# facebookresearch/sam-audio

Measured on AMD Instinct MI355X. Metric: seconds-of-audio separated/sec/node, higher is better.
Workload: dtype fp16x3 (fp32 storage as the reference; every big contraction on IEEE-half hi + lo split operands: 3 MFMA products per multiply, fp32 accumulation - fp32-grade results on the 16-bit matrix cores)

## Files before the change

### sam_audio_amd/csrc/common.h

```cpp
#pragma once
#include <hip/hip_runtime.h>
#include <stdint.h>

namespace sa {

struct bf16_t {
  unsigned short v;
};

#ifdef SA_OPERAND_FP16
__device__ __forceinline__ float bf2f(unsigned short h) { return (float)__builtin_bit_cast(_Float16, h); }
__device__ __forceinline__ unsigned short f2bf(float f) {
  return __builtin_bit_cast(unsigned short, (_Float16)f);
}
__device__ __forceinline__ float h16_lo(unsigned w) { return bf2f((unsigned short)(w & 0xffffu)); }
__device__ __forceinline__ float h16_hi(unsigned w) { return bf2f((unsigned short)(w >> 16)); }
typedef __attribute__((ext_vector_type(8))) _Float16 h16x8_t;
#define SA_MFMA_16x16x32(a, b, c) __builtin_amdgcn_mfma_f32_16x16x32_f16(a, b, c, 0, 0, 0)
#define SA_MFMA_32x32x16(a, b, c) __builtin_amdgcn_mfma_f32_32x32x16_f16(a, b, c, 0, 0, 0)
#else
__device__ __forceinline__ float bf2f(unsigned short h) { return __uint_as_float(((unsigned)h) << 16); }
#ifdef SA_BF16_HW_ROUND
__device__ __forceinline__ unsigned short f2bf(float f) { return __builtin_bit_cast(unsigned short, (__bf16)f); }
#else
__device__ __forceinline__ unsigned short f2bf(float f) {
  unsigned u = __float_as_uint(f);
  u += 0x7fffu + ((u >> 16) & 1u);
  return (unsigned short)(u >> 16);
}
#endif
__device__ __forceinline__ float h16_lo(unsigned w) { return __uint_as_float(w << 16); }
__device__ __forceinline__ float h16_hi(unsigned w) { return __uint_as_float(w & 0xffff0000u); }
typedef __attribute__((ext_vector_type(8))) __bf16 h16x8_t;
#define SA_MFMA_16x16x32(a, b, c) __builtin_amdgcn_mfma_f32_16x16x32_bf16(a, b, c, 0, 0, 0)
#define SA_MFMA_32x32x16(a, b, c) __builtin_amdgcn_mfma_f32_32x32x16_bf16(a, b, c, 0, 0, 0)
#endif

typedef __attribute__((ext_vector_type(2))) float f32x2_t;
#ifdef SA_OPERAND_FP16
typedef __attribute__((ext_vector_type(2))) _Float16 h16x2_t;
#else
typedef __attribute__((ext_vector_type(2))) __bf16 h16x2_t;
#endif
__device__ __forceinline__ unsigned pack_h16x2(float a, float b) {
  const f32x2_t v = {a, b};
  return __builtin_bit_cast(unsigned, __builtin_convertvector(v, h16x2_t));
}

#ifdef SA_OPERAND_FP16
constexpr float kH16Max = 65504.f;
#else
constexpr float kH16Max = 3.3895313892515355e38f;
#endif

__device__ __forceinline__ float clamp_h16(float x) { return fminf(fmaxf(x, -kH16Max), kH16Max); }
struct H16Split { unsigned hi, lo; };
__device__ __forceinline__ H16Split split_h16x2(float v0, float v1) {
#pragma clang fp contract(off)
  const unsigned hi = pack_h16x2(clamp_h16(v0), clamp_h16(v1));
  return H16Split{hi, pack_h16x2(v0 - h16_lo(hi), v1 - h16_hi(hi))};
}

struct alt16_t {
  unsigned short v;
};
typedef __attribute__((ext_vector_type(2))) __bf16 alt16x2_t;
typedef __attribute__((ext_vector_type(8))) __bf16 alt16x8_t;
__device__ __forceinline__ unsigned pack_alt16x2(float a, float b) {
  const f32x2_t v = {a, b};
  return __builtin_bit_cast(unsigned, __builtin_convertvector(v, alt16x2_t));
}
__device__ __forceinline__ unsigned short f2alt(float f) { return (unsigned short)(pack_alt16x2(f, 0.f) & 0xffffu); }
#define SA_MFMA_16x16x32_ALT(a, b, c) \
  __builtin_amdgcn_mfma_f32_16x16x32_bf16(__builtin_bit_cast(alt16x8_t, a), __builtin_bit_cast(alt16x8_t, b), c, 0, 0, 0)

template <typename T> struct Elem;
template <> struct Elem<float> {
  static __device__ __forceinline__ float load(const float* p) { return *p; }
  static __device__ __forceinline__ void store(float* p, float v) { *p = v; }
};
template <> struct Elem<bf16_t> {
  static __device__ __forceinline__ float load(const bf16_t* p) { return bf2f(p->v); }
  static __device__ __forceinline__ void store(bf16_t* p, float v) { p->v = f2bf(v); }
};

template <typename T> __device__ __forceinline__ void store4(T* p, float a, float b, float c, float d);
template <> __device__ __forceinline__ void store4<float>(float* p, float a, float b, float c, float d) {
  *(float4*)p = make_float4(a, b, c, d);
}
template <> __device__ __forceinline__ void store4<bf16_t>(bf16_t* p, float a, float b, float c, float d) {
  ushort4 v;
  v.x = f2bf(a); v.y = f2bf(b); v.z = f2bf(c); v.w = f2bf(d);
  *(ushort4*)p = v;
}
template <> __device__ __forceinline__ void store4<alt16_t>(alt16_t* p, float a, float b, float c, float d) {
  *(uint2*)p = make_uint2(pack_alt16x2(a, b), pack_alt16x2(c, d));
}
template <typename T> __device__ __forceinline__ void load2(const T* p, float& a, float& b);
template <> __device__ __forceinline__ void load2<float>(const float* p, float& a, float& b) {
  float2 v = *(const float2*)p; a = v.x; b = v.y;
}
template <> __device__ __forceinline__ void load2<bf16_t>(const bf16_t* p, float& a, float& b) {
  ushort2 v = *(const ushort2*)p; a = bf2f(v.x); b = bf2f(v.y);
}
template <typename T> __device__ __forceinline__ void store2(T* p, float a, float b);
template <> __device__ __forceinline__ void store2<float>(float* p, float a, float b) { *(float2*)p = make_float2(a, b); }
template <> __device__ __forceinline__ void store2<bf16_t>(bf16_t* p, float a, float b) { *(unsigned*)p = pack_h16x2(a, b); }

__device__ __forceinline__ float silu_f(float x) { return x / (1.0f + __expf(-x)); }
__device__ __forceinline__ float gelu_f(float x) { return 0.5f * x * (1.0f + erff(x * 0.7071067811865476f)); }
__device__ __forceinline__ float quick_gelu_f(float x) { return x / (1.0f + __expf(-1.702f * x)); }
__device__ __forceinline__ float relu_f(float x) { return fmaxf(x, 0.f); }
__device__ __forceinline__ float gelu_tanh_f(float x) {
  return 0.5f * x * (1.0f + tanhf(0.7978845608028654f * (x + 0.044715f * x * x * x)));
}
__device__ __forceinline__ float snake_f(float x, float a) {
  float s = sinf(a * x);
  return x + s * s / (a + 1e-9f);
}
__device__ __forceinline__ float snake16_f(float x, float a) {
  const float s = __sinf(a * x);
  return x + s * s * __builtin_amdgcn_rcpf(a + 1e-9f);
}

template <int CTRL> __device__ __forceinline__ float dpp_mov(float v) {
  return __int_as_float(__builtin_amdgcn_update_dpp(0, __float_as_int(v), CTRL, 0xf, 0xf, false));
}
__device__ __forceinline__ float row16_max(float v) {
  v = fmaxf(v, dpp_mov<0x128>(v));
  v = fmaxf(v, dpp_mov<0x124>(v));
  v = fmaxf(v, dpp_mov<0x122>(v));
  v = fmaxf(v, dpp_mov<0x121>(v));
  return v;
}
__device__ __forceinline__ float row16_sum(float v) {
  v += dpp_mov<0x128>(v);
  v += dpp_mov<0x124>(v);
  v += dpp_mov<0x122>(v);
  v += dpp_mov<0x121>(v);
  return v;
}

__device__ __forceinline__ float wave_sum(float v) {
// ... 64 lines not shown
```

### sam_audio_amd/csrc/gemm.hip

```cpp
#include "common.h"
#include "kernels.h"

#include <type_traits>

namespace sa {

typedef h16x8_t bf16x8_t;
typedef __attribute__((ext_vector_type(4))) float f32x4_t;

template <typename T> struct Mma;
template <> struct Mma<bf16_t> {
  typedef bf16x8_t frag_t;
  static __device__ __forceinline__ f32x4_t run(const frag_t& a, const frag_t& b, f32x4_t c) {
    return SA_MFMA_16x16x32(a, b, c);
  }
};
template <> struct Mma<float> {
  typedef f32x4_t frag_t;
  static __device__ __forceinline__ f32x4_t run(const frag_t& a, const frag_t& b, f32x4_t c) {
    c = __builtin_amdgcn_mfma_f32_16x16x4f32(a[0], b[0], c, 0, 0, 0);
    c = __builtin_amdgcn_mfma_f32_16x16x4f32(a[1], b[1], c, 0, 0, 0);
    c = __builtin_amdgcn_mfma_f32_16x16x4f32(a[2], b[2], c, 0, 0, 0);
    c = __builtin_amdgcn_mfma_f32_16x16x4f32(a[3], b[3], c, 0, 0, 0);
    return c;
// ... 17 lines not shown
  __builtin_amdgcn_global_load_lds((const __attribute__((address_space(1))) void*)gsrc,
                                   (__attribute__((address_space(3))) void*)lds_wave_base, 16, 0, 0);
}

template <typename T, int BM, int BN, int WM_, int WN_, bool FLY = false>
__global__ __launch_bounds__(256, (FLY ? 2 : 1)) void gemm_kernel(const GemmParams p) {
  constexpr int NW = WM_ * WN_;
  static_assert(NW == 4, "4 waves per workgroup");
  constexpr int CH = 16 / (int)sizeof(T);
  constexpr int BK = 128 / (int)sizeof(T);
  constexpr int WTM = BM / WM_, WTN = BN / WN_;
  constexpr int FM = WTM / 16, FN = WTN / 16;
  constexpr int AI = BM / 32, BI = BN / 32;
  static_assert(BM % 32 == 0 && BN % 32 == 0 && WTM % 16 == 0 && WTN % 16 == 0, "tile shape");
  constexpr int TILE_A = BM * 128, TILE_B = BN * 128, STAGE = TILE_A + TILE_B;
  constexpr int NS = 2;
  __shared__ __attribute__((aligned(16))) char smem[NS * STAGE];

  const int tid = threadIdx.x;
  const int lane = tid & 63;
  const int wave = __builtin_amdgcn_readfirstlane(tid >> 6);
  const int wm = wave / WN_, wn = wave % WN_;

  const int tiles_n = (p.N + BN - 1) / BN;
  const int tiles_m = (p.M + BM - 1) / BM;
  int id = blockIdx.x;
  const int tn = id % tiles_n;
  id /= tiles_n;
  const int tm = id % tiles_m;
  const int b = id / tiles_m;
  const int m0 = tm * BM, n0 = tn * BN;

  const int r8 = lane >> 3;
  const int chunk = (lane & 7) ^ ((4 * (wave & 1) + (r8 >> 1)) & 7);
  const T* a_rows[AI];
  const T* w_rows[BI];
  {
    const T* A = (const T*)p.A + p.a_off + (long)b * p.a_bstride;
#pragma unroll
    for (int i = 0; i < AI; ++i) {
      int m = m0 + (wave + 4 * i) * 8 + r8;
      m = m < p.M ? m : p.M - 1;
      a_rows[i] = A + (long)m * p.lda;
    }
    const T* W = (const T*)p.W + (long)b * p.w_bstride;
#pragma unroll
    for (int i = 0; i < BI; ++i) {
      int n = n0 + (wave + 4 * i) * 8 + r8;
      n = n < p.N ? n : p.N - 1;
      w_rows[i] = W + (long)n * p.K + chunk * CH;
    }
  }
  int a_in = chunk * CH;
  long a_tap = 0;
  while (a_in >= p.kc) { a_in -= p.kc; a_tap += p.tap_stride; }

  auto issue = [&](int stage) {
    char* sA = smem + stage * STAGE;
    char* sB = sA + TILE_A;
#pragma unroll
    for (int i = 0; i < AI; ++i) dma16(a_rows[i] + a_tap + a_in, sA + (wave + 4 * i) * 1024);
#pragma unroll
    for (int i = 0; i < BI; ++i) dma16(w_rows[i], sB + (wave + 4 * i) * 1024);
    a_in += BK;
    while (a_in >= p.kc) { a_in -= p.kc; a_tap += p.tap_stride; }
#pragma unroll
    for (int i = 0; i < BI; ++i) w_rows[i] += BK;
  };

  f32x4_t acc[FM][FN];
#pragma unroll
  for (int i = 0; i < FM; ++i)
#pragma unroll
    for (int j = 0; j < FN; ++j) acc[i][j] = f32x4_t{0.f, 0.f, 0.f, 0.f};

  const int nslab = p.K / BK;
  const int lr = lane & 15, lg = lane >> 4;
  const int qa = gemm_quant_a(p.flags), qw = gemm_quant_w(p.flags);
  const bool x3fly = FLY || (sizeof(T) == 4 && (p.flags & GEMM_FLAG_X3_FLY) != 0);
  const bool wfly = FLY || (p.flags & GEMM_FLAG_W_FLY16) != 0;
  auto fly_slab = [&](const char* sA, const char* sB) {
#pragma clang fp contract(off)
        bf16x8_t ah[FM], al[FM], bh[FN], bl[FN];
        auto cl = [](float x) { return __builtin_amdgcn_fmed3f(x, -kH16Max, kH16Max); };
        auto split = [&](const char* base, int row, bf16x8_t& hi, bf16x8_t& lo) {
          const int sw = (row >> 1) & 7;
          const f32x4_t v0 = *(const f32x4_t*)(base + row * 128 + ((lg ^ sw) << 4));
          const f32x4_t v1 = *(const f32x4_t*)(base + row * 128 + (((4 + lg) ^ sw) << 4));
          unsigned h[4], l[4];
          h[0] = pack_h16x2(cl(v0[0]), cl(v0[1]));
          h[1] = pack_h16x2(cl(v0[2]), cl(v0[3]));
          h[2] = pack_h16x2(cl(v1[0]), cl(v1[1]));
          h[3] = pack_h16x2(cl(v1[2]), cl(v1[3]));
          l[0] = pack_h16x2(v0[0] - h16_lo(h[0]), v0[1] - h16_hi(h[0]));
          l[1] = pack_h16x2(v0[2] - h16_lo(h[1]), v0[3] - h16_hi(h[1]));
          l[2] = pack_h16x2(v1[0] - h16_lo(h[2]), v1[1] - h16_hi(h[2]));
          l[3] = pack_h16x2(v1[2] - h16_lo(h[3]), v1[3] - h16_hi(h[3]));
          typedef __attribute__((ext_vector_type(4))) unsigned u32x4_t;
          hi = __builtin_bit_cast(bf16x8_t, (u32x4_t){h[0], h[1], h[2], h[3]});
          lo = __builtin_bit_cast(bf16x8_t, (u32x4_t){l[0], l[1], l[2], l[3]});
        };
        if (wfly) {
#pragma unroll
          for (int j = 0; j < FN; ++j) {
            const int row = wn * WTN + j * 16 + lr, sw = (row >> 1) & 7;
            bh[j] = *(const bf16x8_t*)(sB + row * 128 + ((lg ^ sw) << 4));
            bl[j] = *(const bf16x8_t*)(sB + row * 128 + (((4 + lg) ^ sw) << 4));
          }
        } else {
#pragma unroll
          for (int j = 0; j < FN; ++j) split(sB, wn * WTN + j * 16 + lr, bh[j], bl[j]);
        }
#pragma unroll
        for (int i = 0; i < FM; ++i) split(sA, wm * WTM + i * 16 + lr, ah[i], al[i]);
#pragma unroll
        for (int i = 0; i < FM; ++i)
#pragma unroll
          for (int j = 0; j < FN; ++j) acc[i][j] = SA_MFMA_16x16x32(bh[j], al[i], acc[i][j]);
#pragma unroll
        for (int i = 0; i < FM; ++i)
#pragma unroll
          for (int j = 0; j < FN; ++j) acc[i][j] = SA_MFMA_16x16x32(bl[j], ah[i], acc[i][j]);
#pragma unroll
        for (int i = 0; i < FM; ++i)
#pragma unroll
          for (int j = 0; j < FN; ++j) acc[i][j] = SA_MFMA_16x16x32(bh[j], ah[i], acc[i][j]);
  };
  issue(0);
  for (int s = 0; s < nslab; ++s) {
    asm volatile("s_waitcnt vmcnt(0)" ::: "memory");
    __syncthreads();
    if (s + 1 < nslab) issue((s + 1) & 1);
    const char* sA = smem + (s & 1) * STAGE;
    const char* sB = sA + TILE_A;
    if constexpr (sizeof(T) == 4) {
      if (x3fly) {
        fly_slab(sA, sB);
        continue;
      }
    }
    if constexpr (!FLY) {
#pragma unroll
    for (int ks = 0; ks < 2; ++ks) {
      typename Mma<T>::frag_t af[FM], bfr[FN];
      const int c = ks * 4 + lg;
#pragma unroll
      for (int i = 0; i < FM; ++i) {
        const int row = wm * WTM + i * 16 + lr;
        af[i] = *(const typename Mma<T>::frag_t*)(sA + row * 128 + ((c ^ ((row >> 1) & 7)) << 4));
      }
#pragma unroll
      for (int j = 0; j < FN; ++j) {
        const int row = wn * WTN + j * 16 + lr;
        bfr[j] = *(const typename Mma<T>::frag_t*)(sB + row * 128 + ((c ^ ((row >> 1) & 7)) << 4));
      }
      if constexpr (sizeof(T) == 4) {
        if (qa) {
#pragma unroll
          for (int i = 0; i < FM; ++i) af[i] = quant16x4(af[i], qa);
        }
        if (qw) {
#pragma unroll
          for (int j = 0; j < FN; ++j) bfr[j] = quant16x4(bfr[j], qw);
        }
      }
#pragma unroll
      for (int i = 0; i < FM; ++i)
#pragma unroll
        for (int j = 0; j < FN; ++j) acc[i][j] = Mma<T>::run(bfr[j], af[i], acc[i][j]);
    }
    }
  }

  const long bM = (long)b * p.M;
  const int n_out = p.swiglu ? p.N >> 1 : p.N;
  auto finish = [&](float v, const float bias, const float gate, const float res, const float sa, float& a) -> float {
    v += bias;
    if (p.gate) v *= gate;
    v *= p.alpha;
    v += res;
    a = v;
    if (p.act == ACT_SNAKE) a = snake_f(v, sa);
    else if (p.act == ACT_TANH) a = tanhf(v);
// ... 130 lines not shown
static hipError_t launch_cfg(const GemmParams& p, hipStream_t st) {
  const long tiles = (long)((p.M + BM - 1) / BM) * ((p.N + BN - 1) / BN) * p.nbatch;
  hipLaunchKernelGGL((gemm_kernel<T, BM, BN, WM_, WN_>), dim3((unsigned)tiles), dim3(256), 0, st, p);
  return hipGetLastError();
}

static int g_force = -1;
void gemm_force_variant(int v) { g_force = v; }

const char* gemm_variant_name(int v, bool is_bf16) {
  const GemmVariantRow* r = gemm_variant_row(v);
  return !r ? "" : is_bf16 ? r->name16 : r->name32;
}

static GemmVariant gemm1_variant(const GemmParams& p) {
  const int N = p.N;
  if (p.swiglu) return GV_GEMM_128x128;
  if (N <= 32 || N == 96) return GV_GEMM_128x32;
  if (N <= 64 || (N % 128 != 0 && N % 64 == 0 && N <= 448)) return GV_GEMM_128x64;
  const long t128 = (long)((p.M + 127) / 128) * ((N + 127) / 128) * p.nbatch;
  if (t128 < 192) return 2 * t128 < 192 ? GV_GEMM_128x32 : GV_GEMM_128x64;
  return GV_GEMM_128x128;
}
static GemmVariant fly_variant(const GemmParams& p) {
  if (p.N <= 32) return GV_FLY_128x32;
  if (p.N <= 64) return GV_FLY_128x64;
  if (p.N % 96 == 0 || p.N <= 96) return GV_FLY_128x96;
  return GV_FLY_128x128;
}
int gemm_variant(const GemmParams& p, bool is_bf16) {
  const bool g2 = is_bf16 && gemm2_ok(p);
  if (!is_bf16 && g_force < 0 && (p.flags & GEMM_FLAG_W_FLY16) && debug_flag(DBG_FLY_OLD_TILES) != 1) return fly_variant(p);
  if (g_force > GV_GEMM_128x32) {
    if (g_force == GV_CONV7H && !(g2 && conv7h_ok(p))) return gemm1_variant(p);
    return g2 && gemm_variant_row(g_force) ? g_force : gemm1_variant(p);
  }
  if (g_force >= 0 || !g2) return gemm1_variant(p);
  const long rows256 = (long)((p.M + 255) / 256) * p.nbatch, rows128 = (long)((p.M + 127) / 128) * p.nbatch;
  if (!debug_flag(DBG_NO_CONV7H) && p.N <= 96 && conv7h_ok(p) && rows256 >= 256) return GV_CONV7H;
  if (p.N >= 64 && p.N < 96 && p.K >= 64) return rows256 >= 256 ? GV_GEMM2_256x64_S2 : GV_GEMM2_128x64_K32;
  if (p.N >= 96 && p.N <= 192 && p.K >= 64 && rows128 >= 1024) {
    if (p.N <= 128) return p.K <= 256 ? GV_GEMM2_64x128_K32 : GV_GEMM2_128x128_K32;
    return p.K <= 256 ? GV_GEMM2_128x128_K32 : GV_GEMM2_128x192_K32;
  }
  if (p.N >= 96 && p.K >= 128) {
    if (p.N >= 256) {
      const long t256 = rows256 * ((p.N + 255) / 256);
      if (p.N < 1024 && p.N % 256) return GV_GEMM8S_128x128;
      const long min256 = debug_flag(DBG_GEMM8_MIN_TILES) > 0 ? debug_flag(DBG_GEMM8_MIN_TILES) : 128;
      return t256 >= min256 ? GV_GEMM8_256x256 : GV_GEMM8S_128x128;
    }
    return rows128 * ((p.N + 127) / 128) >= 192 ? GV_GEMM2_128x128_S2 : GV_GEMM2_64x128_S3;
  }
  return gemm1_variant(p);
}

template <typename T>
static hipError_t launch_t(const GemmParams& p, int variant, hipStream_t st) {
  switch (variant) {
    case GV_GEMM_128x32: return launch_cfg<T, 128, 32, 4, 1>(p, st);
    case GV_GEMM_128x64: return launch_cfg<T, 128, 64, 2, 2>(p, st);
    default: return launch_cfg<T, 128, 128, 2, 2>(p, st);
  }
}

int gemm_tail_split(const GemmParams& p, bool is_bf16) {
  if (g_force >= 0 || (p.flags & GEMM_FLAG_NO_TAIL_SPLIT) || gemm_variant(p, is_bf16) != GV_GEMM8_256x256) return 0;
  const long tiles = (long)((p.M + 255) / 256) * ((p.N + 255) / 256) * p.nbatch;
  const long full = tiles / 256 * 256, rem = tiles - full;
  const long min_tail = debug_flag(DBG_TAIL_SPLIT_MIN) > 0 ? debug_flag(DBG_TAIL_SPLIT_MIN) : 8;
  return full >= 256 && full <= 1024 && rem >= min_tail && rem <= 128 ? (int)full : 0;
}
hipError_t launch_gemm_part(const GemmParams& p, bool is_bf16, int part, hipStream_t st) {
  return launch_gemm8_split(p, gemm_tail_split(p, is_bf16), part, st);
}

hipError_t launch_gemm(const GemmParams& p, bool is_bf16, hipStream_t st) {
  if (const int full = gemm_tail_split(p, is_bf16)) {
    const hipError_t e = launch_gemm8_split(p, full, 0, st);
    return e != hipSuccess ? e : launch_gemm8_split(p, full, 1, st);
  }
  const int v = gemm_variant(p, is_bf16);
  if (v >= GV_FLY_128x96) {
    const auto go = [&](auto kern, int bm, int bn) {
      const long tiles = (long)((p.M + bm - 1) / bm) * ((p.N + bn - 1) / bn) * p.nbatch;
      hipLaunchKernelGGL(kern, dim3((unsigned)tiles), dim3(256), 0, st, p);
      return hipGetLastError();
    };
    switch (v) {
      case GV_FLY_128x96: return go(gemm_kernel<float, 128, 96, 4, 1, true>, 128, 96);
      case GV_FLY_128x128: return go(gemm_kernel<float, 128, 128, 4, 1, true>, 128, 128);
      case GV_FLY_128x64: return go(gemm_kernel<float, 128, 64, 4, 1, true>, 128, 64);
      default: return go(gemm_kernel<float, 128, 32, 4, 1, true>, 128, 32);
    }
  }
  if (v > GV_GEMM_128x32) return launch_gemm2(p, (GemmVariant)v, st);
  return is_bf16 ? launch_t<bf16_t>(p, v, st) : launch_t<float>(p, v, st);
}

static const char* need_8phase(const GemmParams& p, bool is_bf16, bool (*eligible)(const GemmParams&), const char* not_eligible,
                               const char* not_chosen) {
  if (!is_bf16 || !gemm2_ok(p) || !eligible(p)) return not_eligible;
  return gemm_is_8phase(gemm_variant(p, is_bf16)) ? nullptr : not_chosen;
}
const char* gemm_check(const GemmParams& p, bool is_bf16) {
  const int bk = is_bf16 ? 64 : 32, ch = is_bf16 ? 8 : 4;
  if (p.M <= 0 || p.N <= 0 || p.K <= 0 || p.nbatch <= 0) return "gemm: empty problem";
  if (p.K % bk) return "gemm: K must be a multiple of 64 (bf16) / 32 (f32) - pad W with zeros";
  if (p.kc % ch || p.kc <= 0) return "gemm: kc must be a positive multiple of the 16-byte chunk";
  if ((p.lda % ch) || (p.tap_stride % ch) || (p.a_off % ch) || (p.a_bstride % ch))
    return "gemm: A strides/offsets must be 16-byte aligned";
  if (p.swiglu && (p.N % 32)) return "gemm: swiglu needs N % 32 == 0";
  if (p.gate && p.rows_per_gate <= 0) return "gemm: rows_per_gate";
  if ((p.flags & GEMM_FLAG_W_FLY16) && (is_bf16 || !(p.flags & GEMM_FLAG_X3_FLY)))
    return "gemm: split-weight layout (flags bit 14): fp32 launches with operands split on the fly (bit 13) only";
  if (p.flags & (GEMM_FLAG_OUT_ALT | GEMM_FLAG_OPND_ALT))
    if (const char* e = need_8phase(p, is_bf16, gemm8_alt_ok, "gemm: alt 16-bit format: plain 16-bit launches with a lean epilogue only",
                                    "gemm: alt 16-bit format: the tile policy did not pick the 8-phase family for this launch")) return e;
  if (p.flags & GEMM_FLAG_OUT_SPLIT3)
    if (const char* e = need_8phase(p, is_bf16, gemm8_split3_ok,
                                    "gemm: split3 output: 16-bit launches with the register epilogue only (SwiGLU, or bias + none / GELU / quick GELU; one 16-bit output, no residual, gate or fp32 output)",
                                    "gemm: split3 output: the tile policy did not pick the 8-phase family for this launch")) return e;
  if (p.flags & GEMM_FLAG_X3_SHARE)
    if (const char* e = need_8phase(p, is_bf16, gemm8_share_ok, "gemm: shared split operands (flags bit 15): plain 16-bit launches with K' = 3K, K % 64 == 0",
                                    "gemm: shared split operands: the tile policy did not pick the 8-phase family for this launch")) return e;
  if (p.flags & GEMM_FLAG_W_KTM)
    if (const char* e = need_8phase(p, is_bf16, [](const GemmParams& q) { return q.w_bstride == 0; },
                                    "gemm: K-tile-major W: plain 16-bit launches with one weight matrix only",
                                    "gemm: K-tile-major W: the tile policy did not pick the 8-phase family for this launch")) return e;
  return nullptr;
}

}
```

### sam_audio_amd/csrc/gemm2.hip

```cpp
#include "common.h"
#include "kernels.h"

namespace sa {

typedef h16x8_t bf16x8_t;
typedef __attribute__((ext_vector_type(16))) float f32x16_t;
typedef __attribute__((ext_vector_type(4))) float f32x4_t;

namespace {

__device__ __forceinline__ void dma16(const void* gsrc, char* lds_wave_base) {
  __builtin_amdgcn_global_load_lds((const __attribute__((address_space(1))) void*)gsrc,
                                   (__attribute__((address_space(3))) void*)lds_wave_base, 16, 0, 0);
}
__device__ __forceinline__ void dma16a(const void* gsrc, char* lds_wave_base) {
  const unsigned lds = __builtin_amdgcn_readfirstlane((unsigned)(size_t)(__attribute__((address_space(3))) char*)lds_wave_base);
  asm volatile("s_mov_b32 m0, %0\n\ts_nop 0\n\tglobal_load_lds_dwordx4 %1, off" ::"s"(lds), "v"(gsrc) : "memory", "m0");
}

template <int N> __device__ __forceinline__ void wait_vmcnt() {
  asm volatile("s_waitcnt vmcnt(%0)" ::"n"(N) : "memory");
}
__device__ __forceinline__ float act_apply(float v, int act, float snake_alpha) {
  if (act == ACT_SILU) return silu_f(v);
  if (act == ACT_GELU) return gelu_f(v);
  if (act == ACT_QUICK_GELU) return quick_gelu_f(v);
  if (act == ACT_RELU) return relu_f(v);
  if (act == ACT_GELU_TANH) return gelu_tanh_f(v);
  if (act == ACT_TANH) return tanhf(v);
  if (act == ACT_SNAKE) return snake16_f(v, snake_alpha);
  return v;
}

}

template <int FM, int FN>
__device__ __forceinline__ void gemm_epilogue_lds(const GemmParams& p, f32x16_t (&acc)[FM][FN], int b, int m_first,
                                                  int n_first, int lane, char* stg) {
  const int l31 = lane & 31, lh = lane >> 5;
  const long bM = (long)b * p.M;
  const bool has_bias = p.bias != nullptr, has_gate = p.gate != nullptr, has_tab = p.gate_tab != nullptr,
             has_res = p.res != nullptr, has_snake = p.act == ACT_SNAKE;
  const int n_out = p.swiglu ? p.N >> 1 : p.N;
  const int cpr = p.swiglu ? FN * 4 : FN * 8;
  const int rb = cpr * 16;
  const int col0 = p.swiglu ? n_first >> 1 : n_first;
  const int units = 32 * cpr;
  const int smask = (cpr & 7) ? 3 : 7;
#pragma unroll
  for (int i = 0; i < FM; ++i) {
#pragma unroll
    for (int j = 0; j < FN; ++j) {
#pragma unroll
      for (int g = 0; g < 4; ++g) {
        float4 v;
        int chunk;
        if (p.swiglu) {
          if (g >= 2) continue;
          v = make_float4(silu_f(acc[i][j][4 * g + 0]) * acc[i][j][4 * (g + 2) + 0],
                          silu_f(acc[i][j][4 * g + 1]) * acc[i][j][4 * (g + 2) + 1],
                          silu_f(acc[i][j][4 * g + 2]) * acc[i][j][4 * (g + 2) + 2],
                          silu_f(acc[i][j][4 * g + 3]) * acc[i][j][4 * (g + 2) + 3]);
          chunk = j * 4 + 2 * g + lh;
        } else {
          v = make_float4(acc[i][j][4 * g + 0], acc[i][j][4 * g + 1], acc[i][j][4 * g + 2], acc[i][j][4 * g + 3]);
          chunk = j * 8 + 2 * g + lh;
        }
        *(float4*)(stg + l31 * rb + ((chunk ^ (l31 & smask)) << 4)) = v;
      }
    }
    asm volatile("s_waitcnt lgkmcnt(0)" ::: "memory");
    for (int u = lane; u < units; u += 64) {
      const int row = u / cpr, chunk = u - row * cpr;
      const float4 sv = *(const float4*)(stg + row * rb + ((chunk ^ (row & smask)) << 4));
      const int m = m_first + i * 32 + row;
      const int n = col0 + chunk * 4;
      const bool m_ok = m < p.M;
      const int mc = m_ok ? m : p.M - 1;
      const int nc = n + 4 <= n_out ? n : n_out - 4;
      const int ch = p.chan_mod ? nc % p.chan_mod : nc;
      float v[4] = {sv.x, sv.y, sv.z, sv.w};
      float4 bb, gg, tt, rr, sa = make_float4(0.f, 0.f, 0.f, 0.f);
      if (has_bias) bb = *(const float4*)(p.bias + ch);
      if (has_gate) gg = *(const float4*)(p.gate + ((bM + mc) / p.rows_per_gate) * p.gate_ld + nc);
// ... 585 lines not shown
    __builtin_amdgcn_s_barrier();
    __builtin_amdgcn_sched_barrier(0);
    auto mid_frags = [&](int kk, bf16x8_t (&mf)[FM]) {
#pragma unroll
      for (int i = 0; i < FM; ++i) mf[i] = *(const bf16x8_t*)(a_lane + kk * 32 + i * 32 * HS);
    };
    mid_frags(0, af[0]);
    mid_frags(1, af[1]);
    __builtin_amdgcn_sched_group_barrier(0x100, 2 * FM, 0);
#pragma unroll
    for (int kk = 0; kk < K1S; ++kk) {
      if (kk + 2 < K1S) mid_frags(kk + 2, af[(kk + 2) % 3]);
#pragma unroll
      for (int i = 0; i < FM; ++i) acc[i] = SA_MFMA_32x32x16(w1[kk], af[kk % 3][i], acc[i]);
      __builtin_amdgcn_sched_group_barrier(0x100, FM, 0);
      __builtin_amdgcn_sched_group_barrier(0x008, FM, 0);
    }
    wait_vmcnt<0>();
#pragma unroll
    for (int i = 0; i < FM; ++i) {
#pragma unroll
      for (int g = 0; g < 4; ++g)
        *(float4*)(stg + l31 * 128 + (((2 * g + lh) ^ (l31 & 7)) << 4)) =
            make_float4(acc[i][4 * g + 0], acc[i][4 * g + 1], acc[i][4 * g + 2], acc[i][4 * g + 3]);
      asm volatile("s_waitcnt lgkmcnt(0)" ::: "memory");
#pragma unroll
      for (int t = 0; t < 4; ++t) {
        const int row = t * 8 + erow;
        const float4 sv = *(const float4*)(stg + row * 128 + (((lane & 7) ^ (row & 7)) << 4));
        const int m = m0 + i * 32 + row;
        float v[4] = {sv.x, sv.y, sv.z, sv.w};
        if (q_bias) { v[0] += qb.x; v[1] += qb.y; v[2] += qb.z; v[3] += qb.w; }
        if (q_res) {
          const float4 rr = *(const float4*)(resb + ((i * 4 + t) * 64 + lane) * 16);
          v[0] += rr.x; v[1] += rr.y; v[2] += rr.z; v[3] += rr.w;
        }
        const float qs[4] = {qsa.x, qsa.y, qsa.z, qsa.w};
        float a[4];
#pragma unroll
        for (int e = 0; e < 4; ++e) a[e] = q_snake ? snake16_f(v[e], qs[e]) : v[e];
        const float a0 = a[0], a1 = a[1], a2 = a[2], a3 = a[3];
        if (m < p.M) {
          if (q.out_f32) {
            float* frow = q.out_f32 + q.f32_off + (long)b * q.f32_bstride + (long)m * q.f32_ld;
            *(float4*)(frow + ncol) = q.f32_act ? make_float4(a0, a1, a2, a3) : make_float4(v[0], v[1], v[2], v[3]);
          }
          bf16_t* arow = (bf16_t*)q.out_act + q.act_off + (long)b * q.act_bstride + (long)m * q.act_ld;
          store4<bf16_t>(arow + ncol, a0, a1, a2, a3);
        }
      }
      asm volatile("s_waitcnt lgkmcnt(0)" ::: "memory");
    }
  }
}

bool conv7h_ok(const GemmParams& p) {
  if (!(p.N == 64 || p.N == 96 || p.N == 128 || p.N == 192)) return false;
  if (p.kc != p.N || p.lda != p.kc || p.w_bstride != 0 || p.swiglu) return false;
  if (p.tap_stride <= 0 || p.tap_stride % p.kc || p.tap_stride / p.kc > 9) return false;
  if (p.K != (7 * p.kc + 63) / 64 * 64) return false;
  return gemm2_ok(p);
}

template <int C, int BM, int WM_, int WN_, int STAGES>
static hipError_t launch_c7(const GemmParams& p, hipStream_t st) {
  const long tiles = (long)((p.M + BM - 1) / BM) * p.nbatch;
  if (p.tag == 1)
    hipLaunchKernelGGL((conv7h_kernel<C, BM, WM_, WN_, STAGES, 1>), dim3((unsigned)tiles), dim3(512), 0, st, p);
  else
    hipLaunchKernelGGL((conv7h_kernel<C, BM, WM_, WN_, STAGES, 0>), dim3((unsigned)tiles), dim3(512), 0, st, p);
  return hipGetLastError();
}

hipError_t launch_conv7h(const GemmParams& p, hipStream_t st) {
  switch (p.N) {
    case 64: return launch_c7<64, 256, 8, 1, 3>(p, st);
    case 96: return launch_c7<96, 256, 8, 1, 3>(p, st);
    case 128: return launch_c7<128, 256, 4, 2, 3>(p, st);
    case 192: return launch_c7<192, 128, 4, 2, 3>(p, st);
    default: return hipErrorInvalidValue;
  }
}

bool resunit_ok(const GemmParams& p, const GemmParams& q) {
  if (!conv7h_ok(p) || !gemm2_ok(q)) return false;
  if (q.N != p.N || q.M != p.M || q.nbatch != p.nbatch || q.kc != p.N || q.lda != p.N || q.w_bstride != 0) return false;
  if (q.K != (p.N + 63) / 64 * 64 || q.swiglu || q.gate || q.chan_mod || q.c_ld_rel || q.alpha != 1.f) return false;
  if (p.gate || p.chan_mod || p.c_ld_rel || p.res || p.out_f32 || p.f32_act || !p.out_act) return false;
  if (p.act != ACT_SNAKE && p.act != ACT_NONE) return false;
  if (q.A != p.out_act || q.a_off != p.act_off || q.a_bstride != p.act_bstride || p.act_ld != p.N) return false;
  if (!q.out_act || q.out_act == p.A) return false;
  return true;
}

template <int C, int BM, int WM_, int WN_, int STAGES>
static hipError_t launch_ru(const GemmParams& p, const GemmParams& q, hipStream_t st) {
  const long tiles = (long)((p.M + BM - 1) / BM) * p.nbatch;
  if (p.tag == 1)
    hipLaunchKernelGGL((resunit_kernel<C, BM, WM_, WN_, STAGES, 1>), dim3((unsigned)tiles), dim3(WM_ * WN_ * 64), 0, st, p, q);
  else
    hipLaunchKernelGGL((resunit_kernel<C, BM, WM_, WN_, STAGES, 0>), dim3((unsigned)tiles), dim3(WM_ * WN_ * 64), 0, st, p, q);
  return hipGetLastError();
}

template <int C>
static hipError_t launch_ws(const GemmParams& p, const GemmParams& q, long tiles, hipStream_t st) {
  const long cap = debug_flag(DBG_RESUNIT_WS) == DBG_WS_ALWAYS_GRID3 ? 3 : 256;
  const unsigned grid = (unsigned)(tiles < cap ? tiles : cap);
  if (p.tag == 1)
    hipLaunchKernelGGL((resws_kernel<C, 1>), dim3(grid), dim3(C / 32 * 64), 0, st, p, q);
  else
    hipLaunchKernelGGL((resws_kernel<C, 0>), dim3(grid), dim3(C / 32 * 64), 0, st, p, q);
  return hipGetLastError();
}

static bool resunit_ws(const GemmParams& p, const GemmParams& q) {
  if (!(p.N == 64 || p.N == 96) || debug_flag(DBG_RESUNIT_WS) == DBG_WS_NEVER) return false;
  if (q.act != ACT_SNAKE && q.act != ACT_NONE) return false;
  if (debug_flag(DBG_RESUNIT_WS) == DBG_WS_ALWAYS || debug_flag(DBG_RESUNIT_WS) == DBG_WS_ALWAYS_GRID3) return true;
  return p.N == 96 && (long)((p.M + 127) / 128) * p.nbatch >= 1024;
}

hipError_t launch_resunit(const GemmParams& p, const GemmParams& q, hipStream_t st) {
  if (resunit_ws(p, q)) {
    const long tiles = (long)((p.M + 127) / 128) * p.nbatch;
    return p.N == 64 ? launch_ws<64>(p, q, tiles, st) : launch_ws<96>(p, q, tiles, st);
  }
  switch (p.N) {
    case 64: return launch_ru<64, 256, 8, 1, 3>(p, q, st);
    case 96: return launch_ru<96, 128, 4, 1, 2>(p, q, st);
    case 128: return launch_ru<128, 256, 4, 2, 3>(p, q, st);
    case 192: return launch_ru<192, 128, 4, 2, 3>(p, q, st);
    default: return hipErrorInvalidValue;
  }
}

template <int BM, int BN, int WM_, int WN_, int STAGES, int BK, bool TAGGED = false>
static hipError_t launch2(const GemmParams& p, hipStream_t st) {
  const long tiles = (long)((p.M + BM - 1) / BM) * ((p.N + BN - 1) / BN) * p.nbatch;
  if (TAGGED && p.tag == 1)
    hipLaunchKernelGGL((gemm2_kernel<BM, BN, WM_, WN_, STAGES, BK, TAGGED ? 1 : 0>), dim3((unsigned)tiles),
                       dim3(WM_ * WN_ * 64), 0, st, p);
  else
    hipLaunchKernelGGL((gemm2_kernel<BM, BN, WM_, WN_, STAGES, BK, 0>), dim3((unsigned)tiles), dim3(WM_ * WN_ * 64), 0,
                       st, p);
  return hipGetLastError();
}

bool gemm2_ok(const GemmParams& p) {
  if ((p.chan_mod & 3) || (p.c_ld_rel & 3) || (p.c_lo & 3) || (p.c_hi & 3)) return false;
  if (p.act == ACT_SNAKE && (!p.act_alpha || ((uintptr_t)p.act_alpha & 15))) return false;
  if (p.N % 4 || p.K % 64) return false;
  if (p.swiglu && p.N % 32) return false;
  auto al4 = [](long v) { return (v & 3) == 0; };
  if (p.out_f32 && !(al4(p.f32_ld) && al4(p.f32_off) && al4(p.f32_bstride) && ((uintptr_t)p.out_f32 & 15) == 0))
    return false;
  if (p.out_act && !(al4(p.act_ld) && al4(p.act_off) && al4(p.act_bstride) && ((uintptr_t)p.out_act & 7) == 0))
    return false;
  if (p.res && !(al4(p.res_ld) && al4(p.res_off) && al4(p.res_bstride) && ((uintptr_t)p.res & 15) == 0)) return false;
  if (p.gate && !(al4(p.gate_ld) && ((uintptr_t)p.gate & 15) == 0)) return false;
  if (p.gate_tab && ((uintptr_t)p.gate_tab & 15)) return false;
  if (p.bias && ((uintptr_t)p.bias & 15)) return false;
  return true;
}

hipError_t launch_gemm2(const GemmParams& p, GemmVariant variant, hipStream_t st) {
// ... 17 lines not shown
```

### sam_audio_amd/csrc/kernels.h

```cpp
#pragma once
#include "common.h"

namespace sa {

hipError_t launch_poison_lds(hipStream_t st);

enum DebugFlag : int {
  DBG_NO_CONV7H = 11,
  DBG_RESUNIT_TWO_LAUNCHES = 16,
  DBG_RESUNIT_FUSE_ALWAYS = 18,
  DBG_RESUNIT_WS = 19,
  DBG_GEMM8S_PLAIN = 21,
  DBG_GEMM8_EPILOGUE = 24,
  DBG_GEMM8_NOT_PERSISTENT = 26,
  DBG_GEMM8S_ROLES = 27,
  DBG_QKV_PREP_SWROUND = 29,
  DBG_GEMM8_MIN_TILES = 30,
  DBG_FOLD_PER_LAYER = 31,
  DBG_TAIL_SPLIT_MIN = 33,
  DBG_RASTER_GM = 35,
  DBG_FLY_OLD_TILES = 36,
  DBG_X3_PLAIN_WALK = 38,
};
enum : int { DBG_WS_ALWAYS = 1, DBG_WS_NEVER = 2, DBG_WS_ALWAYS_GRID3 = 3 };
enum : int { DBG_EPI_GENERAL = 1, DBG_EPI_LINEAR = 2, DBG_EPI_ROWS = 3 };
enum : int { DBG_ROLES_NONE = 1, DBG_ROLES_PROD0 = 2, DBG_ROLES_PROD2 = 3 };
void set_debug_flag(int flag, int value);
hipError_t launch_hash_items(const unsigned* x, size_t words_per_item, int items, unsigned long long* out, hipStream_t st);
constexpr int kSentinelPartials = 256;
hipError_t launch_sentinel(const void* x, int fmt, long rows, int cols, long ld, float* partial, float* slot, hipStream_t st);
__attribute__((weak)) bool sentinel_built();
void* debug_device_alloc(size_t bytes);
void debug_device_free(void* p);
int debug_flag(int flag);

hipError_t launch_gemm(const GemmParams& p, bool is_bf16, hipStream_t st);
const char* gemm_check(const GemmParams& p, bool is_bf16);
enum GemmVariant : int {
  GV_GEMM_128x128 = 0,
  GV_GEMM_128x64 = 1,
  GV_GEMM_128x32 = 2,
  GV_GEMM8_256x256 = 22,
  GV_GEMM8S_128x128 = 27,
  GV_GEMM2_128x128_S2 = 25,
  GV_GEMM2_64x128_S3 = 26,
  GV_GEMM2_256x64_S2 = 28,
  GV_GEMM2_128x128_K32 = 29,
  GV_GEMM2_128x64_K32 = 32,
  GV_GEMM2_64x128_K32 = 33,
  GV_GEMM2_128x192_K32 = 34,
  GV_CONV7H = 35,
  GV_FLY_128x96 = 36,
  GV_FLY_128x128 = 37,
  GV_FLY_128x64 = 38,
  GV_FLY_128x32 = 39,
};
constexpr int kGemmVariants = 40;
enum GemmFamily : int { FAM_TILES, FAM_32x32x16, FAM_8PHASE, FAM_FLY };
struct GemmVariantRow {
  GemmVariant id;
  GemmFamily family;
  const char* name16;
  const char* name32;
};
inline constexpr GemmVariantRow kGemmVariantTable[] = {
    {GV_GEMM_128x128, FAM_TILES, "gemm_bf16_128x128", "gemm_f32_128x128"},
    {GV_GEMM_128x64, FAM_TILES, "gemm_bf16_128x64", "gemm_f32_128x64"},
    {GV_GEMM_128x32, FAM_TILES, "gemm_bf16_128x32", "gemm_f32_128x32"},
    {GV_GEMM8_256x256, FAM_8PHASE, "gemm8_bf16_256x256_8phase", ""},
    {GV_GEMM2_128x128_S2, FAM_32x32x16, "gemm2_bf16_128x128_s2", ""},
    {GV_GEMM2_64x128_S3, FAM_32x32x16, "gemm2_bf16_64x128_s3", ""},
    {GV_GEMM8S_128x128, FAM_8PHASE, "gemm8s_bf16_128x128", ""},
    {GV_GEMM2_256x64_S2, FAM_32x32x16, "gemm2_bf16_256x64_s2", ""},
    {GV_GEMM2_128x128_K32, FAM_32x32x16, "gemm2_bf16_128x128_k32_s3", ""},
    {GV_GEMM2_128x64_K32, FAM_32x32x16, "gemm2_bf16_128x64_k32_s2", ""},
    {GV_GEMM2_64x128_K32, FAM_32x32x16, "gemm2_bf16_64x128_k32_s3", ""},
    {GV_GEMM2_128x192_K32, FAM_32x32x16, "gemm2_bf16_128x192_k32_s3", ""},
    {GV_CONV7H, FAM_32x32x16, "conv7h_bf16", ""},
    {GV_FLY_128x96, FAM_FLY, "", "gemm_f32x3_128x96"},
    {GV_FLY_128x128, FAM_FLY, "", "gemm_f32x3_128x128"},
    {GV_FLY_128x64, FAM_FLY, "", "gemm_f32x3_128x64"},
    {GV_FLY_128x32, FAM_FLY, "", "gemm_f32x3_128x32"},
};
constexpr const GemmVariantRow* gemm_variant_row(int v) {
  for (const GemmVariantRow& r : kGemmVariantTable)
    if (r.id == v) return &r;
  return nullptr;
}
constexpr bool gemm_is_8phase(int v) { return gemm_variant_row(v) && gemm_variant_row(v)->family == FAM_8PHASE; }
constexpr const char* kGemm8sTailName = "gemm8s_bf16_128x128_tail";
int gemm_variant(const GemmParams& p, bool is_bf16);
const char* gemm_variant_name(int variant, bool is_bf16);
bool gemm2_ok(const GemmParams& p);
hipError_t launch_gemm2(const GemmParams& p, GemmVariant variant, hipStream_t st);
hipError_t launch_gemm8(const GemmParams& p, hipStream_t st);
bool gemm8_share_ok(const GemmParams& p);
hipError_t launch_gemm8s(const GemmParams& p, hipStream_t st);
bool gemm8_alt_ok(const GemmParams& p);
bool gemm8_split3_ok(const GemmParams& p);
bool conv7h_ok(const GemmParams& p);
hipError_t launch_conv7h(const GemmParams& p, hipStream_t st);
bool resunit_ok(const GemmParams& p, const GemmParams& q);
hipError_t launch_resunit(const GemmParams& p, const GemmParams& q, hipStream_t st);
hipError_t launch_gemm8_split(const GemmParams& p, int full, int part, hipStream_t st);
int gemm_tail_split(const GemmParams& p, bool is_bf16);
hipError_t launch_gemm_part(const GemmParams& p, bool is_bf16, int part, hipStream_t st);
void gemm_force_variant(int v);

hipError_t launch_rmsnorm_mod(const float* x, const float* w, const float* shift_tab, const float* scale_tab,
                              const float* tvec, long tvec_ld, int shift_off, int scale_off, void* out, bool bf16,
                              int M, int D, int rows_per_b, float eps, hipStream_t st);

hipError_t launch_layernorm_accum(const float* x, const float* w, const float* b, const float* gate, float* acc,
                                  int M, int D, float eps, hipStream_t st);

hipError_t launch_groupnorm_silu(const float* x, const float* w, const float* b, double* partials, void* out,
                                 bool bf16, int B, int T, int C, int halo, float eps, hipStream_t st);

constexpr int kMaxModNorms = 96;
struct ModTables {
  const float* w[kMaxModNorms];
  const float* shift_tab[kMaxModNorms];
  const float* scale_tab[kMaxModNorms];
  int shift_off[kMaxModNorms], scale_off[kMaxModNorms];
};
hipError_t launch_mod_tables(const ModTables& t, int n_norms, const float* tvec, long tvec_ld, int nt, float* gs, int D,
                             hipStream_t st);
hipError_t launch_rmsnorm_gs(const float* x, const float* gs, long gs_ld, void* out, bool bf16, int M, int D, int rows_per_b,
                             float eps, hipStream_t st, bool out_alt = false);
hipError_t launch_rmsnorm_gs_split3(const float* x, const float* gs, long gs_ld, void* out, int M, int D, int rows_per_b, float eps,
                                    hipStream_t st);
hipError_t launch_qkv_prep(const void* qkv, const float* qw, const float* kw, const float* rope_cos,
                           const float* rope_sin, void* Q, void* K, void* Vt, bool bf16, int B, int T, int Tp, int H,
                           float eps, hipStream_t st, int head_dim = 128);

hipError_t launch_qkv_prep_f32x(const float* qkv, const float* qw, const float* kw, const float* rope_cos, const float* rope_sin, float* Q,
                                float* K, float* Vt, int B, int T, int Tp, int H, float eps, hipStream_t st);

hipError_t launch_self_attention(const void* Q, const void* K, const void* Vt, const unsigned char* key_mask,
                                 void* out, bool bf16, int B, int T, int Tp, int H, hipStream_t st, bool out_alt = false);

hipError_t launch_self_attention_hd(const void* Q, const void* K, const void* Vt, const unsigned char* key_mask,
                                    void* out, bool bf16, int B, int T, int Tp, int H, int head_dim, hipStream_t st,
                                    bool out_alt = false);

hipError_t launch_self_attention_x3(const float* Q, const float* K, const float* Vt, const unsigned char* key_mask, float* out,
                                    int B, int T, int Tp, int H, int head_dim, hipStream_t st, void* out3 = nullptr);

hipError_t launch_headnorm(void* x, const float* w, bool bf16, int rows, long ld, int col0, int H, float eps,
                           hipStream_t st, int head_dim = 128);

hipError_t launch_cross_attention(const void* q, const float* qw, const void* kv, long kv_ld,
                                  const unsigned char* mask, void* out, bool bf16, int B, int T, int Lt, int H,
                                  float eps, hipStream_t st, int head_dim = 128);
hipError_t launch_cross_attn_probs(const void* q, const float* qw, const void* kv, long kv_ld, const unsigned char* mask,
                                   void* P, int ldp, int B, int T, int Lt, int LtP, int H, float eps, hipStream_t st);
hipError_t launch_cross_attn_fold(const void* wo, const void* kv, long kv_ld, void* UT, int KP, int B, int Lt, int LtP,
                                  int H, hipStream_t st);
constexpr int kMaxFoldLayers = 48;
hipError_t launch_cross_attn_fold_layers(const void* const* wo, int n_layers, const void* kv_all, long kv_ld, void* UT_all, int KP,
                                         int B, int Lt, int LtP, int H, hipStream_t st);
hipError_t launch_cross_attn_probs3(const float* q, const float* qw, const float* kv, long kv_ld, const unsigned char* mask, void* P3,
                                    int KP, int B, int T, int Lt, int LtP, int H, float eps, hipStream_t st);
hipError_t launch_cross_attn_fold3_layers(const float* const* wo, int n_layers, const float* kv_all, long kv_ld, void* UT3_all, int KP,
                                          int B, int Lt, int LtP, int H, hipStream_t st);
hipError_t launch_headnorm_layers(void* kv_all, const float* w_all, bool bf16, int rows, int L, int H, float eps,
                                  hipStream_t st, int head_dim = 128);

hipError_t launch_time_features(const float* t, int nt, const float* freqs, int fdim, const float* inv_freq, int D,
                                void* temb, float* tsin, bool bf16, hipStream_t st);

struct FloatPack {
  static constexpr int N = 64;
  float v[N];
};
hipError_t launch_set_floats(float* dst, const float* host_values, int n, hipStream_t st);

struct OdeStageArgs {
  const float* k[4];
  float coef[4];
  int n_src;
};
__attribute__((weak)) hipError_t launch_ode_stage(const float* y0, const OdeStageArgs& a, float scale, float* out, long n,
                                                  hipStream_t st);
// ... 145 lines not shown
```

Measured before the change: 94.97.

## Add fly7 kernel for 7-tap dilated convs with split-once A halo tile

Adds a specialized kernel for 7-tap dilated convolution GEMMs with 64 or 96 channels. It splits the input activation halo into fp16 hi/lo once into LDS and reuses that tile across all 7 taps, while weights stream through a multi-stage async ring. The old path re-split A on the fly for every slab, so this targets the repeated split ALU work and redundant A loads. It also fuses bias, residual and snake into the epilogue and moves the shared split into a helper in common.h. In exchange it uses a larger LDS footprint and adds another specialized code path, with the old tiles still reachable through a debug flag.

```diff
diff --git a/sam_audio_amd/csrc/common.h b/sam_audio_amd/csrc/common.h
--- a/sam_audio_amd/csrc/common.h
+++ b/sam_audio_amd/csrc/common.h
@@ -59,6 +59,24 @@
 #pragma clang fp contract(off)
   const unsigned hi = pack_h16x2(clamp_h16(v0), clamp_h16(v1));
   return H16Split{hi, pack_h16x2(v0 - h16_lo(hi), v1 - h16_hi(hi))};
+}
+
+typedef __attribute__((ext_vector_type(4))) float f32x4_t;
+__device__ __forceinline__ void fly_split8(const f32x4_t v0, const f32x4_t v1, h16x8_t& hi, h16x8_t& lo) {
+#pragma clang fp contract(off)
+  auto cl = [](float x) { return __builtin_amdgcn_fmed3f(x, -kH16Max, kH16Max); };
+  unsigned h[4], l[4];
+  h[0] = pack_h16x2(cl(v0[0]), cl(v0[1]));
+  h[1] = pack_h16x2(cl(v0[2]), cl(v0[3]));
+  h[2] = pack_h16x2(cl(v1[0]), cl(v1[1]));
+  h[3] = pack_h16x2(cl(v1[2]), cl(v1[3]));
+  l[0] = pack_h16x2(v0[0] - h16_lo(h[0]), v0[1] - h16_hi(h[0]));
+  l[1] = pack_h16x2(v0[2] - h16_lo(h[1]), v0[3] - h16_hi(h[1]));
+  l[2] = pack_h16x2(v1[0] - h16_lo(h[2]), v1[1] - h16_hi(h[2]));
+  l[3] = pack_h16x2(v1[2] - h16_lo(h[3]), v1[3] - h16_hi(h[3]));
+  typedef __attribute__((ext_vector_type(4))) unsigned u32x4_t;
+  hi = __builtin_bit_cast(h16x8_t, (u32x4_t){h[0], h[1], h[2], h[3]});
+  lo = __builtin_bit_cast(h16x8_t, (u32x4_t){l[0], l[1], l[2], l[3]});
 }
 
 struct alt16_t {
diff --git a/sam_audio_amd/csrc/gemm.hip b/sam_audio_amd/csrc/gemm.hip
--- a/sam_audio_amd/csrc/gemm.hip
+++ b/sam_audio_amd/csrc/gemm.hip
@@ -123,23 +123,9 @@
   auto fly_slab = [&](const char* sA, const char* sB) {
 #pragma clang fp contract(off)
         bf16x8_t ah[FM], al[FM], bh[FN], bl[FN];
-        auto cl = [](float x) { return __builtin_amdgcn_fmed3f(x, -kH16Max, kH16Max); };
         auto split = [&](const char* base, int row, bf16x8_t& hi, bf16x8_t& lo) {
           const int sw = (row >> 1) & 7;
-          const f32x4_t v0 = *(const f32x4_t*)(base + row * 128 + ((lg ^ sw) << 4));
-          const f32x4_t v1 = *(const f32x4_t*)(base + row * 128 + (((4 + lg) ^ sw) << 4));
-          unsigned h[4], l[4];
-          h[0] = pack_h16x2(cl(v0[0]), cl(v0[1]));
-          h[1] = pack_h16x2(cl(v0[2]), cl(v0[3]));
-          h[2] = pack_h16x2(cl(v1[0]), cl(v1[1]));
-          h[3] = pack_h16x2(cl(v1[2]), cl(v1[3]));
-          l[0] = pack_h16x2(v0[0] - h16_lo(h[0]), v0[1] - h16_hi(h[0]));
-          l[1] = pack_h16x2(v0[2] - h16_lo(h[1]), v0[3] - h16_hi(h[1]));
-          l[2] = pack_h16x2(v1[0] - h16_lo(h[2]), v1[1] - h16_hi(h[2]));
-          l[3] = pack_h16x2(v1[2] - h16_lo(h[3]), v1[3] - h16_hi(h[3]));
-          typedef __attribute__((ext_vector_type(4))) unsigned u32x4_t;
-          hi = __builtin_bit_cast(bf16x8_t, (u32x4_t){h[0], h[1], h[2], h[3]});
-          lo = __builtin_bit_cast(bf16x8_t, (u32x4_t){l[0], l[1], l[2], l[3]});
+          fly_split8(*(const f32x4_t*)(base + row * 128 + ((lg ^ sw) << 4)), *(const f32x4_t*)(base + row * 128 + (((4 + lg) ^ sw) << 4)), hi, lo);
         };
         if (wfly) {
 #pragma unroll
@@ -436,6 +422,7 @@
   }
   const int v = gemm_variant(p, is_bf16);
   if (v >= GV_FLY_128x96) {
+    if (debug_flag(DBG_FLY_OLD_TILES) != 2 && fly7_ok(p)) return launch_fly7(p, st);
     const auto go = [&](auto kern, int bm, int bn) {
       const long tiles = (long)((p.M + bm - 1) / bm) * ((p.N + bn - 1) / bn) * p.nbatch;
       hipLaunchKernelGGL(kern, dim3((unsigned)tiles), dim3(256), 0, st, p);
diff --git a/sam_audio_amd/csrc/gemm2.hip b/sam_audio_amd/csrc/gemm2.hip
--- a/sam_audio_amd/csrc/gemm2.hip
+++ b/sam_audio_amd/csrc/gemm2.hip
@@ -1,5 +1,7 @@
 #include "common.h"
 #include "kernels.h"
+
+#include <type_traits>
 
 namespace sa {
 
@@ -751,6 +753,230 @@
   }
 }
 
+template <int C, int NW, int FM, int DIL, int STAGES>
+__global__ __launch_bounds__(NW * 64, 2) void fly7_kernel(const GemmParams p) {
+  constexpr int BM = NW * FM * 16, FN = C / 16;
+  constexpr int SL = C / 32;
+  constexpr int HR = (BM + 6 * DIL + 15) / 16 * 16;
+  constexpr int PLANE = HR * 16, TILE = SL * 8 * PLANE;
+  constexpr int WQ = C / 8, BI = (WQ + NW - 1) / NW;
+  constexpr int TILE_W = C * 128;
+  constexpr int LDS = TILE + STAGES * TILE_W;
+  static_assert(C % 32 == 0 && NW % 2 == 0 && WQ >= NW, "tile shape");
+  static_assert(LDS <= 160 * 1024, "LDS budget");
+  static_assert(BM * C * 4 <= LDS, "epilogue staging fits");
+  static_assert((STAGES - 2) * BI <= 63, "vmcnt range");
+  __shared__ __attribute__((aligned(16))) char smem[LDS];
+  char* const tile = smem;
+  char* const ring = smem + TILE;
+
+  const int tid = threadIdx.x;
+  const int lane = tid & 63;
+  const int wave = __builtin_amdgcn_readfirstlane(tid >> 6);
+
+  const int tiles_m = (p.M + BM - 1) / BM;
+  int b, tm;
+  {
+    const int total = tiles_m * p.nbatch;
+    const int bid = blockIdx.x;
+    const int q = total >> 3, r = total & 7;
+    const int xcd = bid & 7, idx = bid >> 3;
+    const int L = (xcd < r ? xcd * (q + 1) : r * (q + 1) + (xcd - r) * q) + idx;
+    b = L / tiles_m;
+    tm = L - b * tiles_m;
+  }
+  const int m0 = tm * BM;
+
+  const int r8 = lane >> 3;
+  const int wchunk = (lane & 7) ^ ((4 * (wave & 1) + (r8 >> 1)) & 7);
+  const int my_bi = (WQ - wave + NW - 1) / NW;
+  const float* w_rows[BI];
+  {
+    const float* W = (const float*)p.W + (long)b * p.w_bstride;
+#pragma unroll
+    for (int i = 0; i < BI; ++i) {
+      int n = (wave + NW * i) * 8 + r8;
+      n = n < C ? n : C - 1;
+      w_rows[i] = W + (long)n * p.K + wchunk * 4;
+    }
+  }
+  auto issue = [&](int stage) {
+    char* sB = ring + stage * TILE_W;
+#pragma unroll
+    for (int i = 0; i < BI; ++i)
+      if (i < my_bi) dma16a(w_rows[i], sB + (wave + NW * i) * 1024);
+#pragma unroll
+    for (int i = 0; i < BI; ++i) w_rows[i] += 32;
+  };
+  auto wait_slab = [&](bool more_in_flight) {
+    if (STAGES > 2 && more_in_flight) {
+      if (my_bi == BI) wait_vmcnt<(STAGES - 2) * BI>();
+      else wait_vmcnt<(STAGES - 2) * (BI - 1)>();
+    } else {
+      wait_vmcnt<0>();
+    }
+  };
+  const int nslab = 7 * SL;
+#pragma unroll
+  for (int s = 0; s < STAGES - 1; ++s) issue(s);
+
+  {
+    const float* A = (const float*)p.A + p.a_off + (long)b * p.a_bstride;
+    const int last_row = p.M - 1 + 6 * DIL;
+    const int rs = (lane & 7) + 8 * (lane >> 5), c = (lane >> 3) & 3;
+    constexpr int UNITS = (HR / 16) * SL, U = (UNITS + NW - 1) / NW;
+    static_assert(U <= 8, "staging batch: 8 registers per unit");
+    f32x4_t v0[U], v1[U];
+#pragma unroll
+    for (int k = 0; k < U; ++k) {
+      const int u = wave + k * NW < UNITS ? wave + k * NW : UNITS - 1;
+      const int rb = u / SL, j = u - rb * SL;
+      int mr = m0 + rb * 16 + rs;
+      mr = mr < last_row ? mr : last_row;
+      const float* src = A + (long)mr * C + j * 32 + c * 4;
+      v0[k] = *(const f32x4_t*)src;
+      v1[k] = *(const f32x4_t*)(src + 16);
+    }
+#pragma unroll
+    for (int k = 0; k < U; ++k) {
+      const int u = wave + k * NW;
+      if (u < UNITS) {
+        const int rb = u / SL, j = u - rb * SL;
+        bf16x8_t hi, lo;
+        fly_split8(v0[k], v1[k], hi, lo);
+        char* dst = tile + (j * 8 + c) * PLANE + (rb * 16 + rs) * 16;
+        *(bf16x8_t*)dst = hi;
+        *(bf16x8_t*)(dst + 4 * PLANE) = lo;
+      }
+    }
+    asm volatile("s_waitcnt lgkmcnt(0)" ::: "memory");
+  }
+
+  f32x4_t acc[FM][FN];
+#pragma unroll
+  for (int i = 0; i < FM; ++i)
+#pragma unroll
+    for (int j = 0; j < FN; ++j) acc[i][j] = f32x4_t{0.f, 0.f, 0.f, 0.f};
+  const int lr = lane & 15, lg = lane >> 4;
+  const char* const a_lane = tile + lg * PLANE + (wave * FM * 16 + lr) * 16;
+  const int b_hi = lr * 128 + ((lg ^ ((lr >> 1) & 7)) << 4), b_lo = b_hi ^ 64;
+
+  int st_c = 0, st_i = (STAGES - 1) % STAGES, tap = 0, js = 0;
+  for (int s = 0; s < nslab; ++s) {
+    wait_slab(s + STAGES - 2 < nslab);
+    __builtin_amdgcn_s_barrier();
+    __builtin_amdgcn_sched_barrier(0);
+    if (s + STAGES - 1 < nslab) issue(st_i);
+    const char* sB = ring + st_c * TILE_W;
+    const char* a_k = a_lane + js * 8 * PLANE + tap * (DIL * 16);
+    bf16x8_t ah[FM], al[FM], bh[FN], bl[FN];
+#pragma unroll
+    for (int i = 0; i < FM; ++i) al[i] = *(const bf16x8_t*)(a_k + 4 * PLANE + i * 256);
+#pragma unroll
+    for (int j = 0; j < FN; ++j) bh[j] = *(const bf16x8_t*)(sB + b_hi + j * 2048);
+#pragma unroll
+    for (int i = 0; i < FM; ++i) ah[i] = *(const bf16x8_t*)(a_k + i * 256);
+#pragma unroll
+    for (int j = 0; j < FN; ++j) bl[j] = *(const bf16x8_t*)(sB + b_lo + j * 2048);
+#pragma unroll
+    for (int i = 0; i < FM; ++i)
+#pragma unroll
+      for (int j = 0; j < FN; ++j) acc[i][j] = SA_MFMA_16x16x32(bh[j], al[i], acc[i][j]);
+#pragma unroll
+    for (int i = 0; i < FM; ++i)
+#pragma unroll
+      for (int j = 0; j < FN; ++j) acc[i][j] = SA_MFMA_16x16x32(bl[j], ah[i], acc[i][j]);
+#pragma unroll
+    for (int i = 0; i < FM; ++i)
+#pragma unroll
+      for (int j = 0; j < FN; ++j) acc[i][j] = SA_MFMA_16x16x32(bh[j], ah[i], acc[i][j]);
+    st_c = st_c + 1 == STAGES ? 0 : st_c + 1;
+    st_i = st_i + 1 == STAGES ? 0 : st_i + 1;
+    if (++js == SL) { js = 0; ++tap; }
+  }
+
+  constexpr int CPR = C / 4, RPI = 64 / CPR, WR = BM / NW, NIT = (WR + RPI - 1) / RPI;
+  __syncthreads();
+#pragma unroll
+  for (int i = 0; i < FM; ++i)
+#pragma unroll
+    for (int j = 0; j < FN; ++j) {
+      const int row = (wave * FM + i) * 16 + lr, c = j * 4 + lg;
+      *(f32x4_t*)(smem + row * (C * 4) + ((c ^ (row & 7)) << 4)) = acc[i][j];
+    }
+  __syncthreads();
+  const int c = lane % CPR, rsub = lane / CPR;
+  const bool lane_on = rsub < RPI;
+  const int n = c * 4;
+  float4 bb = make_float4(0.f, 0.f, 0.f, 0.f), sa = bb;
+  if (p.bias) bb = *(const float4*)(p.bias + n);
+  if (p.act == ACT_SNAKE) sa = *(const float4*)(p.act_alpha + n);
+  const float* const res0 = p.res ? p.res + p.res_off + (long)b * p.res_bstride + n : nullptr;
+  float* const f320 = p.out_f32 ? p.out_f32 + p.f32_off + (long)b * p.f32_bstride + n : nullptr;
+  float* const act0 = p.out_act ? (float*)p.out_act + p.act_off + (long)b * p.act_bstride + n : nullptr;
+  const int rw = wave * WR;
+  auto body = [&](auto SNAKE) {
+    auto fin = [&](float v, const float bias, const float res, const float sal, float& a) -> float {
+      v += bias;
+      v *= p.alpha;
+      v += res;
+      a = decltype(SNAKE)::value ? snake_f(v, sal) : v;
+      return v;
+    };
+    auto res_of = [&](int it) {
+      const int m = m0 + rw + it * RPI + rsub;
+      float4 r = make_float4(0.f, 0.f, 0.f, 0.f);
+      if (res0) r = *(const float4*)(res0 + (long)(m < p.M ? m : p.M - 1) * p.res_ld);
+      return r;
+    };
+    float4 rr = res_of(0);
+#pragma unroll 1
+    for (int it = 0; it < NIT; ++it) {
+      float4 rn = make_float4(0.f, 0.f, 0.f, 0.f);
+      if (it + 1 < NIT) rn = res_of(it + 1);
+      const int rl = it * RPI + rsub, row = rw + (rl < WR ? rl : 0), m = m0 + row;
+      const float4 sv = *(const float4*)(smem + row * (C * 4) + ((c ^ (row & 7)) << 4));
+      float a0, a1, a2, a3;
+      const float v0 = fin(sv.x, bb.x, rr.x, sa.x, a0), v1 = fin(sv.y, bb.y, rr.y, sa.y, a1), v2 = fin(sv.z, bb.z, rr.z, sa.z, a2),
+                  v3 = fin(sv.w, bb.w, rr.w, sa.w, a3);
+      if (lane_on && rl < WR && m < p.M) {
+        if (f320) *(float4*)(f320 + (long)m * p.f32_ld) = p.f32_act ? make_float4(a0, a1, a2, a3) : make_float4(v0, v1, v2, v3);
+        if (act0) *(float4*)(act0 + (long)m * p.act_ld) = make_float4(a0, a1, a2, a3);
+      }
+      rr = rn;
+    }
+  };
+  if (p.act == ACT_SNAKE) body(std::true_type{});
+  else body(std::false_type{});
+}
+
+bool fly7_ok(const GemmParams& p) {
+  constexpr int want = GEMM_FLAG_X3_FLY | GEMM_FLAG_W_FLY16;
+  if ((p.flags & want) != want || p.M <= 0 || p.nbatch <= 0) return false;
+  if (!(p.N == 64 || p.N == 96)) return false;
+  if (p.kc != p.N || p.lda != p.kc || p.K != 7 * p.kc) return false;
+  if (!(p.tap_stride == p.kc || p.tap_stride == 3 * p.kc || (p.tap_stride == 9 * p.kc && p.N == 96))) return false;
+  if (p.swiglu || p.gate || p.chan_mod || p.c_ld_rel || (p.act != ACT_NONE && p.act != ACT_SNAKE)) return false;
+  auto al16 = [](const void* q, long a, long b, long c) { return (((size_t)q) & 15) == 0 && !((a | b | c) & 3); };
+  return al16(p.A, p.a_off, p.a_bstride, p.w_bstride) && al16(p.W, 0, 0, 0) && (!p.bias || al16(p.bias, 0, 0, 0)) &&
+         (p.act != ACT_SNAKE || (p.act_alpha && al16(p.act_alpha, 0, 0, 0))) && (!p.res || al16(p.res, p.res_off, p.res_ld, p.res_bstride)) &&
+         (!p.out_f32 || al16(p.out_f32, p.f32_off, p.f32_ld, p.f32_bstride)) && (!p.out_act || al16(p.out_act, p.act_off, p.act_ld, p.act_bstride));
+}
+
+template <int C, int NW, int FM, int DIL, int STAGES>
+static hipError_t launch_f7(const GemmParams& p, hipStream_t st) {
+  constexpr int BM = NW * FM * 16;
+  const long tiles = (long)((p.M + BM - 1) / BM) * p.nbatch;
+  hipLaunchKernelGGL((fly7_kernel<C, NW, FM, DIL, STAGES>), dim3((unsigned)tiles), dim3(NW * 64), 0, st, p);
+  return hipGetLastError();
+}
+hipError_t launch_fly7(const GemmParams& p, hipStream_t st) {
+  if (!fly7_ok(p)) return hipErrorInvalidValue;
+  const int dil = (int)(p.tap_stride / p.kc);
+  if (p.N == 64) return dil == 1 ? launch_f7<64, 4, 2, 1, 3>(p, st) : launch_f7<64, 4, 2, 3, 3>(p, st);
+  return dil == 1 ? launch_f7<96, 4, 2, 1, 2>(p, st) : dil == 3 ? launch_f7<96, 8, 2, 3, 3>(p, st) : launch_f7<96, 8, 2, 9, 3>(p, st);
+}
+
 bool resunit_ok(const GemmParams& p, const GemmParams& q) {
   if (!conv7h_ok(p) || !gemm2_ok(q)) return false;
   if (q.N != p.N || q.M != p.M || q.nbatch != p.nbatch || q.kc != p.N || q.lda != p.N || q.w_bstride != 0) return false;
diff --git a/sam_audio_amd/csrc/kernels.h b/sam_audio_amd/csrc/kernels.h
--- a/sam_audio_amd/csrc/kernels.h
+++ b/sam_audio_amd/csrc/kernels.h
@@ -100,6 +100,8 @@
 bool gemm8_split3_ok(const GemmParams& p);
 bool conv7h_ok(const GemmParams& p);
 hipError_t launch_conv7h(const GemmParams& p, hipStream_t st);
+bool fly7_ok(const GemmParams& p);
+hipError_t launch_fly7(const GemmParams& p, hipStream_t st);
 bool resunit_ok(const GemmParams& p, const GemmParams& q);
 hipError_t launch_resunit(const GemmParams& p, const GemmParams& q, hipStream_t st);
 hipError_t launch_gemm8_split(const GemmParams& p, int full, int part, hipStream_t st);
```

Measured after the change: 95.05 (median of 6 runs). No clear change (+0.1%).
